# zhanggefan/mmdet3d-gaussian

Measured on AMD Instinct MI355X. Metric: M box-pairs/sec (fwd+bwd) for GWD/KLD/BCD @10M pairs, higher is better.
Workload: dtype f32; 1 GPU; 10000000 synthetic anchor x gt 7-dof box pairs per GPU (BASELINE configs[2]); step = gwd3d + kld3d + bd3d, each GDLoss forward + backward over the whole batch (one plain backward() of the summed losses; fun=log1p, tau=1, reduction=mean, loss_weight=5); pairs_per_gpu=10000000, parallelism=pair-sharded x1, launch=eager, gc_disabled=True, input_allocation=one torch allocation per array, device=MI355X (HIP kernels)

## Files before the change

### include/gd3d.h

```cpp
#ifndef GD3D_H_
#define GD3D_H_

#include <stddef.h>
#include <stdint.h>

#ifdef __cplusplus
extern "C" {
#endif

#define GD3D_ABI_VERSION 6

#define GD3D_E_BADARG 10001
#define GD3D_E_TOOLARGE 10002
#define GD3D_E_HOST 10003

enum {
  GD3D_GWD3D = 0,
  GD3D_KLD3D = 1,
  GD3D_BD3D = 2,
  GD3D_JD3D = 3,
  GD3D_KLD3D_SYMMAX = 4,
  GD3D_KLD3D_SYMMIN = 5,
  GD3D_KFIOU3D = 6,
  GD3D_NUM_LOSS_TYPES = 7
// ... 113 lines not shown
                           int32_t n_l1, float* losses, void* workspace, void* stream);
int gd3d_center_head_keys(int32_t num_tasks, int64_t max_n, int64_t* byte_offset, int64_t* byte_stride);
int gd3d_center_head_finish(const gd3d_params* params, const gd3d_prologue* coder,
                            const gd3d_center_task* tasks, int32_t num_tasks, const float* code_weights,
                            int32_t n_l1, float* losses, void* workspace, const int64_t* order,
                            void* stream);

int gd3d_loss_fused_select(const gd3d_params* params, const gd3d_prologue* prologue, const float* pred,
                           const float* target, const float* weight7, int64_t n, float scale,
                           float* loss_sum, int32_t* any_positive, float* grad_pred, float* grad_target,
                           void* workspace, void* stream, void* start_event, void* stop_event);

int64_t gd3d_one_launch_max_n(void);
int gd3d_loss_fused_one_launch(const gd3d_params* params, const gd3d_prologue* prologue, const float* pred,
                               const float* target, const float* row_weight, const float* weight7, int64_t n,
                               float scale, float* loss_sum, int32_t* any_positive, float* grad_pred,
                               float* grad_target, void* workspace, int32_t* ticket, void* stream);

size_t gd3d_loss_fused_multi_workspace_bytes(int32_t count, int64_t n);
int gd3d_loss_fused_multi_eligible(const gd3d_params* params);
int gd3d_loss_fused_multi(int32_t count, const gd3d_params* params, const float* const* preds, const float* target,
                          int64_t n, const float* scales, float* const* loss_sums, float* const* grad_preds,
                          void* workspace, void* stream);

int gd3d_grad_finish(float* grad_pred, float* grad_target, const float* g, int64_t n,
                     const int32_t* any_positive, const float* weight7, const float* pred,
                     const gd3d_prologue* prologue, void* stream);

int gd3d_probe_stream(const float* x, const float* y, float* z, int64_t n_floats, void* stream,
                      void* start_event, void* stop_event);

int coder_center_decode(const gd3d_prologue* coder, const float* locs, const float* preds, int64_t n,
                        int32_t c, int32_t correct_yaw, float* out, int32_t* num_rot_parity, void* stream);

int coder_center_decode_backward(const gd3d_prologue* coder, const float* grad_out, const float* out,
                                 const int32_t* num_rot_parity, int64_t n, int32_t c,
                                 float* grad_preds, void* stream);

int coder_center_encode(const float* boxes, int64_t n, int32_t c, float* out, void* stream);

int coder_point_decode(const float* priors, const float* preds, int64_t n, int32_t c, int32_t correct_yaw, float* out,
                       int32_t* num_rot_parity, void* stream);
int coder_point_decode_backward(const float* priors, const float* grad_out, const float* out,
                                const int32_t* num_rot_parity, int64_t n, int32_t c, float* grad_preds, void* stream);

int coder_roi_decode(const float* rois, int32_t roi_stride, int32_t first_col, const float* bbox_pred, int64_t n,
// ... 445 lines not shown
```

### mmdet3d-gaussian_amd/_lib.py

```python
import ctypes
import os

from . import build as _build

_lib = None


class Params(ctypes.Structure):
    _fields_ = [('loss_type', ctypes.c_int32), ('fun', ctypes.c_int32),
                ('tau', ctypes.c_float), ('alpha', ctypes.c_float),
                ('center_offset', ctypes.c_float * 3), ('flag', ctypes.c_int32)]


class Prologue(ctypes.Structure):
    _fields_ = [('kind', ctypes.c_int32), ('norm_bbox', ctypes.c_int32), ('aux', ctypes.c_void_p),
                ('out_size_factor', ctypes.c_float), ('voxel_size', ctypes.c_float * 2),
                ('pc_range', ctypes.c_float * 2), ('reserved', ctypes.c_float)]


def fill_geometry(struct, coder):
    struct.norm_bbox = int(bool(coder.norm_bbox))
    struct.out_size_factor = float(coder.out_size_factor)
    struct.voxel_size = (ctypes.c_float * 2)(float(coder.voxel_size[0]), float(coder.voxel_size[1]))
    struct.pc_range = (ctypes.c_float * 2)(float(coder.pc_range[0]), float(coder.pc_range[1]))
# ... 74 lines not shown
                ('gt_start', ctypes.c_int32 * 65), ('pos_iou_thr', ctypes.c_float * 16), ('neg_iou_thr', ctypes.c_float * 16),
                ('min_pos_iou', ctypes.c_float * 16), ('pos_weight', ctypes.c_float), ('dir_offset', ctypes.c_float)]


_vp, _i64, _f32, _int, _sz = ctypes.c_void_p, ctypes.c_int64, ctypes.c_float, ctypes.c_int, ctypes.c_size_t
_i32 = ctypes.c_int32
SYMBOLS = {
    'gd3d_loss_workspace_bytes': (_sz, [_i64]),
    'gd3d_loss_fused': (_int, [ctypes.POINTER(Params), _vp, _vp, _vp, _i64, _f32, _vp, _vp, _vp, _vp, _vp, _vp]),
    'gd3d_loss_fused_w7': (_int, [ctypes.POINTER(Params), _vp, _vp, _vp, _vp, _i64, _f32, _vp, _vp, _vp, _vp, _vp, _vp]),
    'gd3d_loss_fused_decoded': (_int, [ctypes.POINTER(Params), ctypes.POINTER(Prologue), _vp, _vp, _vp, _vp, _i64, _f32,
                                       _vp, _vp, _vp, _vp, _vp, _vp]),
    'gd3d_loss_fused_timed': (_int, [ctypes.POINTER(Params), ctypes.POINTER(Prologue), _vp, _vp, _vp, _vp, _i64, _f32,
                                     _vp, _vp, _vp, _vp, _vp, _vp, _vp, _vp]),
    'gd3d_loss_fused_select': (_int, [ctypes.POINTER(Params), ctypes.POINTER(Prologue), _vp, _vp, _vp, _i64, _f32, _vp, _vp,
                                      _vp, _vp, _vp, _vp, _vp, _vp]),
    'gd3d_one_launch_max_n': (_i64, []),
    'gd3d_loss_fused_one_launch': (_int, [ctypes.POINTER(Params), ctypes.POINTER(Prologue), _vp, _vp, _vp, _vp, _i64, _f32, _vp, _vp,
                                          _vp, _vp, _vp, _vp, _vp]),
    'gd3d_loss_fused_multi_workspace_bytes': (_sz, [_i32, _i64]),
    'gd3d_loss_fused_multi_eligible': (_int, [ctypes.POINTER(Params)]),
    'gd3d_loss_fused_multi': (_int, [_i32, ctypes.POINTER(Params), ctypes.POINTER(_vp), _vp, _i64, ctypes.POINTER(_f32),
                                     ctypes.POINTER(_vp), ctypes.POINTER(_vp), _vp, _vp]),
    'gd3d_loss_fused_cpu': (_int, [ctypes.POINTER(Params), _vp, _vp, _vp, _vp, _i64, _f32, _vp, _vp, _vp, _vp, _vp, ctypes.c_int32]),
    'gd3d_loss_reduce_cpu': (_int, [_vp, _i64, _vp]),
    'gd3d_scale_rows_cpu': (_int, [_vp, _vp, _int, _i64, ctypes.c_int32]),
    'riou_bev_xyxyr_cpu': (_int, [_vp, _i64, _vp, _i64, _vp, ctypes.c_int32]),
    'riou_eval_bev_cpu': (_int, [_vp, _i64, _vp, _i64, _vp, ctypes.c_int32]),
    'riou_eval_3d_cpu': (_int, [_vp, _i64, _vp, _i64, _f32, _vp, ctypes.c_int32]),
    'riou_eval_trans_bev_cpu': (_int, [_vp, _i64, ctypes.c_int32, _vp, _i64, ctypes.c_int32, _vp, ctypes.c_int32]),
    'rnms_bev_cpu': (_int, [_vp, _i64, _f32, _vp, _vp]),
    'rnms_normal_bev_cpu': (_int, [_vp, _i64, _f32, _vp, _vp]),
    'gd3d_grad_finish': (_int, [_vp, _vp, _vp, _i64, _vp, _vp, _vp, ctypes.POINTER(Prologue), _vp]),
    'gd3d_probe_stream': (_int, [_vp, _vp, _vp, _i64, _vp, _vp, _vp]),
    'gd3d_prof_event_create': (_int, [ctypes.POINTER(_vp)]),
    'gd3d_prof_event_destroy': (_int, [_vp]),
    'gd3d_prof_event_elapsed_ms': (_int, [_vp, _vp, ctypes.POINTER(ctypes.c_float)]),
    'gd3d_anchor_head_loss': (_int, [ctypes.POINTER(Params), _vp, ctypes.c_int32, ctypes.c_int32, ctypes.c_int32,
                                     ctypes.c_int32, _vp, _vp, ctypes.POINTER(ctypes.c_float), _vp, _vp, _i64, _f32, _vp,
                                     _vp, _vp, _vp]),
    'gd3d_anchor_head_loss_dense': (_int, [ctypes.POINTER(Params), _vp, ctypes.c_int32, ctypes.c_int32, ctypes.c_int32,
                                           ctypes.c_int32, _vp, _vp, ctypes.POINTER(ctypes.c_float), _vp, _vp,
                                           ctypes.c_int32, _f32, _vp, _vp, _vp, _vp]),
    'gd3d_anchor_head_bbox_loss': (_int, [ctypes.POINTER(Params), ctypes.POINTER(SmoothL1), _vp, ctypes.c_int32,
                                          ctypes.c_int32, ctypes.c_int32, ctypes.c_int32, _vp, _vp,
                                          ctypes.POINTER(ctypes.c_float), _vp, _vp, _i64, _vp, ctypes.c_int32, _f32, _vp,
# ... 421 lines not shown
```

### mmdet3d-gaussian_amd/build.py

```python
import concurrent.futures
import hashlib
import os
import shutil
import subprocess

PKG_DIR = os.path.dirname(os.path.abspath(__file__))
CSRC = os.path.join(PKG_DIR, 'csrc')
LIB_PATH = os.path.join(PKG_DIR, 'libgd3d.so')
ARCH = 'gfx950'

SOURCES = {
    'gd3d_loss.hip': ['-fno-hip-fp32-correctly-rounded-divide-sqrt', '-ffp-contract=fast'],
    'gd3d_anchor_head.hip': ['-fno-hip-fp32-correctly-rounded-divide-sqrt', '-ffp-contract=fast'],
    'gd3d_center_head.hip': ['-fno-hip-fp32-correctly-rounded-divide-sqrt', '-ffp-contract=fast'],
    'rbox.hip': ['-ffp-contract=off'],
    'voxel_scatter.hip': [],
    'device_sort.hip': [],
    'voxel_index.hip': [],
    'eval_match.hip': ['-ffp-contract=off'],
    'coders.hip': ['-ffp-contract=off'],
    'vsa.hip': ['-ffp-contract=off'],
    'pib.hip': ['-ffp-contract=off'],
    'roi_head.hip': ['-ffp-contract=off'],
    'roi_sample.hip': ['-ffp-contract=off'],
# ... 132 lines not shown
          main_objs
    r = subprocess.run(cmd, capture_output=True, text=True)
    if r.returncode != 0:
        raise RuntimeError(f'link failed:\n{r.stderr[-4000:]}')
    os.replace(tmp, LIB_PATH)
    tmp = f'{EXTRAS_PATH}.{os.getpid()}.tmp'
    cmd = [hipcc, '--offload-arch=' + ARCH, '-shared', '-fPIC', '-pthread', '-o', tmp] + extra_objs + \
          ['-L' + PKG_DIR, '-l:libgd3d.so', '-Wl,-rpath,$ORIGIN']
    r = subprocess.run(cmd, capture_output=True, text=True)
    if r.returncode != 0:
        raise RuntimeError(f'link of libgd3d_extras.so failed:\n{r.stderr[-4000:]}')
    os.replace(tmp, EXTRAS_PATH)
    with open(HASH_PATH + f'.{os.getpid()}', 'w') as f:
        f.write(source_hash())
    os.replace(HASH_PATH + f'.{os.getpid()}', HASH_PATH)
    shutil.rmtree(objdir, ignore_errors=True)
    return LIB_PATH


def node_source_hash():
    import torch
    h = hashlib.sha256()
    h.update(torch.__version__.encode())
    for d in (os.path.join(CSRC, NODE_SOURCE), os.path.join(PKG_DIR, '..', 'include', 'gd3d.h')):
        with open(d, 'rb') as f:
            h.update(f.read())
    h.update(repr(node_command('OUT', cxx='CXX')).encode())
    return h.hexdigest()


def node_command(out, cxx=None):
    import sysconfig
    import torch
    tdir = os.path.dirname(os.path.abspath(torch.__file__))
    tlib = os.path.join(tdir, 'lib')
    return [cxx or host_cxx_path(), '-std=c++17', '-O2', '-fPIC', '-shared', '-Wall', '-Wno-unused-function',
            '-D__HIP_PLATFORM_AMD__=1', '-DUSE_ROCM=1', '-DTORCH_EXTENSION_NAME=_gd3d_node',
            f'-D_GLIBCXX_USE_CXX11_ABI={int(torch._C._GLIBCXX_USE_CXX11_ABI)}',
            '-isystem', os.path.join(tdir, 'include'), '-isystem', os.path.join(tdir, 'include', 'torch', 'csrc', 'api', 'include'),
            '-isystem', '/opt/rocm/include', '-isystem', sysconfig.get_paths()['include'],
            os.path.join(CSRC, NODE_SOURCE), '-o', out,
            '-L' + tlib, '-ltorch', '-ltorch_cpu', '-lc10', '-lc10_hip', '-ltorch_hip', '-ltorch_python', '-ldl',
            '-Wl,-rpath,' + tlib]


def node_is_stale():
    if not os.path.isfile(NODE_PATH) or not os.path.isfile(NODE_HASH_PATH):
# ... 28 lines not shown
```

### mmdet3d-gaussian_amd/csrc/gd3d_loss.hip

```cpp
#include <hip/hip_ext.h>

#include <mutex>
#include <unordered_map>

#include "gd3d_loss_common.h"

namespace gd3d {

constexpr int TILE = 256;
constexpr int TILE_F = TILE * 7;
constexpr int TILE_V4 = TILE_F / 4;
constexpr int NPIECE = TILE_F / 256;
constexpr int NWAVE = TILE / 64;

typedef __attribute__((address_space(3))) void lds_ptr_t;
typedef const __attribute__((address_space(1))) void gbl_cptr_t;

constexpr int DMA_AUX = 2;
constexpr int DMA_AUX_TARGET = 0;
constexpr int MIN_LDS = 27300;
constexpr int MIN_LDS_GWD = 32768;
constexpr int MIN_LDS_W7 = 32768;
constexpr int MIN_LDS_KLD = MIN_LDS;
constexpr int MIN_LDS_BD = MIN_LDS;
// ... 440 lines not shown
    double s2 = 0.0;
#pragma unroll
    for (int k = 0; k < 16; ++k) s2 += sd[tid * 16 + k];
#pragma unroll
    for (int off = 32; off >= 1; off >>= 1) s2 += __shfl_down(s2, off, 64);
    if (tid == 0) *out = (float)s2;
  }
}
__global__ __launch_bounds__(1024) void reduce_partials_kernel(const float* __restrict__ partials, long long nb,
                                                               float* __restrict__ out) {
  __shared__ double sd[1024];
  reduce_partials_body(partials, nb, out, sd);
}
struct ReduceMultiArgs {
  float* out[MULTI_MAX];
};
__global__ __launch_bounds__(1024) void reduce_partials_multi_kernel(const float* __restrict__ partials, long long nb,
                                                                     long long nbp, const ReduceMultiArgs o) {
  __shared__ double sd[1024];
  float* out = o.out[0];
  if (blockIdx.x == 1) out = o.out[1];
  if (blockIdx.x == 2) out = o.out[2];
  reduce_partials_body(partials + (long long)blockIdx.x * nbp, nb, out, sd);
}
int reduce_partials(const float* partials, long long nb, float* out, hipStream_t s) {
  hipLaunchKernelGGL(reduce_partials_kernel, dim3(1), dim3(1024), 0, s, partials, nb, out);
  return (int)hipGetLastError();
}

__global__ __launch_bounds__(1024) void scale_rows_kernel(float* __restrict__ grad, const float* __restrict__ g,
                                                         int per_row, long long nflt) {
  float gs = 1.0f;
  if (!per_row) {
    gs = g[0];
    if (gs == 1.0f) return;
  }
  const long long stride = (long long)gridDim.x * blockDim.x;
  const long long i0 = (long long)blockIdx.x * blockDim.x + threadIdx.x;
  if (!per_row && (((uintptr_t)grad & 15) == 0)) {
    v4f* g4 = reinterpret_cast<v4f*>(grad);
    const long long nv = nflt >> 2;
    for (long long i = i0; i < nv; i += stride) g4[i] = g4[i] * gs;
    for (long long i = (nv << 2) + i0; i < nflt; i += stride) grad[i] *= gs;
    return;
  }
  for (long long i = i0; i < nflt; i += stride) grad[i] *= per_row ? g[i / 7] : gs;
// ... 359 lines not shown
  hipExtLaunchKernelGGL(probe_add_kernel, dim3((unsigned)nb), dim3(PROBE_T), 0u, (hipStream_t)stream, (hipEvent_t)start_event,
                        (hipEvent_t)stop_event, 0u, (const v4f*)x, (const v4f*)y, (v4f*)z, nv);
  return (int)hipGetLastError();
}

int gd3d_loss_reduce(const void* workspace, int64_t n, float* loss_sum, void* stream) {
  if (n < 0 || loss_sum == nullptr) return GD3D_E_BADARG;
  hipStream_t s = (hipStream_t)stream;
  if (n == 0) return fill_words(loss_sum, sizeof(float), 0u, s);
  if (workspace == nullptr) return GD3D_E_BADARG;
  const long long nparts = (n + TILE - 1) / TILE;
  return reduce_partials((const float*)workspace, nparts, loss_sum, s);
}

size_t gd3d_loss_fused_multi_workspace_bytes(int32_t count, int64_t n) {
  if (n <= 0 || count <= 0) return 64;
  return (size_t)(4 * (int64_t)count * ws_nbp(n) + 16);
}

int gd3d_loss_fused_multi_eligible(const gd3d_params* p) {
  return p != nullptr && multi_marked(p->loss_type, p->fun, p->flag != 0) ? 1 : 0;
}

int gd3d_loss_fused_multi(int32_t count, const gd3d_params* params, const float* const* preds, const float* target,
                          int64_t n, const float* scales, float* const* loss_sums, float* const* grad_preds,
                          void* workspace, void* stream) {
  if (count < 2 || count > MULTI_MAX || params == nullptr || preds == nullptr || scales == nullptr || loss_sums == nullptr ||
      n < 0)
    return GD3D_E_BADARG;
  for (int k = 0; k < count; ++k) {
    if (!gd3d_loss_fused_multi_eligible(&params[k]) || loss_sums[k] == nullptr) return GD3D_E_BADARG;
    if (n > 0 && preds[k] == nullptr) return GD3D_E_BADARG;
  }
  hipStream_t s = (hipStream_t)stream;
  if (n == 0) {
    for (int k = 0; k < count; ++k) {
      const int e0 = fill_words(loss_sums[k], sizeof(float), 0u, s);
      if (e0 != 0) return e0;
    }
    return 0;
  }
  if (target == nullptr || workspace == nullptr || ((uintptr_t)workspace & 15) != 0) return GD3D_E_BADARG;
  const int64_t nb = (n + TILE - 1) / TILE;
  if (nb > 0x7fffffffLL) return GD3D_E_TOOLARGE;
  int order[MULTI_MAX] = {0, 1, 2};
  for (int i = 1; i < count; ++i)
    for (int j = i; j > 0 && params[order[j]].loss_type < params[order[j - 1]].loss_type; --j) {
      const int t = order[j];
      order[j] = order[j - 1];
      order[j - 1] = t;
    }
  const long long nbp = ws_nbp(n);
  MultiArgs a = {};
  ReduceMultiArgs r = {};
  uintptr_t bits = (uintptr_t)target;
  int lt[MULTI_MAX] = {-1, -1, -1};
  for (int j = 0; j < count; ++j) {
    const int k = order[j];
    const gd3d_params& p = params[k];
    lt[j] = p.loss_type;
// ... 3 lines not shown
    a.scale[j] = scales[k];
    a.alpha[j] = p.alpha;
    a.ia2[j] = gd3d_inv_alpha2(p.alpha);
    a.tau[j] = p.tau;
    for (int q = 0; q < 3; ++q) a.c[j][q] = p.center_offset[q];
    r.out[j] = loss_sums[k];
    bits |= (uintptr_t)a.pred[j] | (uintptr_t)a.gp[j];
  }
  a.target = target;
  a.n = n;
  a.vec_ok = (bits & 15) == 0;
  bool reuse = false;
  next_tile_order_reversed(s, nullptr, -1, &reuse);
  const hipError_t e = with_multi_tuple(lt[0], lt[1], lt[2], [&](auto tup) {
    using T = decltype(tup);
    constexpr int K = T::count;
    size_t lds = (size_t)((K + 1) * TILE_F + 32) * sizeof(float);
    constexpr size_t min_lds = K == 3 ? MULTI_LDS_K3 : MULTI_LDS_K2;
    if (lds < min_lds) lds = min_lds;
    hipLaunchKernelGGL((fused_multi_kernel<T::l0, T::l1, T::l2>), dim3((unsigned)nb), dim3(TILE), lds, s, a);
    return hipGetLastError();
  });
  if (e != hipSuccess) return (int)e;
  hipLaunchKernelGGL(reduce_partials_multi_kernel, dim3((unsigned)count), dim3(1024), 0, s, (const float*)workspace,
                     (long long)nb, nbp, r);
  return (int)hipGetLastError();
}

int gd3d_prof_event_create(void** event) {
  if (event == nullptr) return GD3D_E_BADARG;
  hipEvent_t e = nullptr;
  const hipError_t rc = hipEventCreate(&e);
  *event = (void*)e;
  return (int)rc;
}

int gd3d_prof_event_destroy(void* event) {
  if (event == nullptr) return 0;
  return (int)hipEventDestroy((hipEvent_t)event);
}

int gd3d_prof_event_elapsed_ms(void* start_event, void* stop_event, float* ms) {
  if (start_event == nullptr || stop_event == nullptr || ms == nullptr) return GD3D_E_BADARG;
  return (int)hipEventElapsedTime(ms, (hipEvent_t)start_event, (hipEvent_t)stop_event);
}

int gd3d_scale_rows(float* grad, const float* g, int per_row, int64_t n, void* stream) {
  if (n < 0 || (n > 0 && (grad == nullptr || g == nullptr))) return GD3D_E_BADARG;
  if (n == 0) return 0;
// ... 15 lines not shown
```

### mmdet3d-gaussian_amd/csrc/torch_node.cpp

```cpp
#include <torch/extension.h>
#include <torch/csrc/autograd/functions/basic_ops.h>
#include <torch/csrc/autograd/functions/utils.h>
#include <torch/csrc/autograd/saved_variable.h>
#include <c10/hip/HIPStream.h>
#include <ATen/Parallel.h>

#include <dlfcn.h>

#include <atomic>
#include <chrono>
#include <cstring>
#include <exception>
#include <limits>
#include <mutex>
#include <sstream>
#include <vector>

#include "../../include/gd3d.h"

namespace {

using at::Tensor;
using torch::autograd::variable_list;

struct Abi {
  decltype(&::gd3d_loss_fused_decoded) loss_fused_decoded = nullptr;
  decltype(&::gd3d_loss_fused_timed) loss_fused_timed = nullptr;
  decltype(&::gd3d_loss_fused_select) loss_fused_select = nullptr;
  decltype(&::gd3d_loss_fused_one_launch) loss_fused_one_launch = nullptr;
  decltype(&::gd3d_loss_fused_multi) loss_fused_multi = nullptr;
  decltype(&::gd3d_loss_fused_multi_eligible) loss_fused_multi_eligible = nullptr;
  decltype(&::gd3d_loss_fused_multi_workspace_bytes) loss_fused_multi_workspace_bytes = nullptr;
  decltype(&::gd3d_grad_finish) grad_finish = nullptr;
  decltype(&::gd3d_loss_fused_cpu) loss_fused_cpu = nullptr;
  decltype(&::gd3d_scale_rows_cpu) scale_rows_cpu = nullptr;
  decltype(&::gd3d_abi_version) abi_version = nullptr;
  decltype(&::rnms_scored) nms_scored = nullptr;
  decltype(&::gd3d_anchor_head_bbox_loss) anchor_head = nullptr;
  decltype(&::gd3d_anchor_head_bbox_loss_dyn) anchor_head_dyn = nullptr;
  decltype(&::gd3d_scale_rows) scale_rows = nullptr;
  decltype(&::gd3d_loss_workspace_bytes) loss_workspace_bytes = nullptr;
  decltype(&::vox_scatter_reduce) scatter_reduce = nullptr;
  decltype(&::vox_scatter_backward) scatter_backward = nullptr;
  decltype(&::vox_scatter_backward_grouped) scatter_backward_grouped = nullptr;
  decltype(&::rnms_scored_workspace_bytes) nms_scored_workspace_bytes = nullptr;
  bool bound = false;
} abi;

template <typename F>
void resolve(void* image, const char* name, F& slot) {
  slot = reinterpret_cast<F>(dlsym(image, name));
  TORCH_CHECK(slot != nullptr, "gd3d node: libgd3d.so does not export ", name);
}

int bind(const std::string& path) {
  void* image = dlopen(path.c_str(), RTLD_NOW | RTLD_LOCAL);
  TORCH_CHECK(image != nullptr, "gd3d node: cannot open ", path, ": ", dlerror());
  resolve(image, "gd3d_loss_fused_decoded", abi.loss_fused_decoded);
  resolve(image, "gd3d_loss_fused_timed", abi.loss_fused_timed);
  resolve(image, "gd3d_loss_fused_select", abi.loss_fused_select);
  resolve(image, "gd3d_loss_fused_one_launch", abi.loss_fused_one_launch);
  resolve(image, "gd3d_loss_fused_multi", abi.loss_fused_multi);
  resolve(image, "gd3d_loss_fused_multi_eligible", abi.loss_fused_multi_eligible);
  resolve(image, "gd3d_loss_fused_multi_workspace_bytes", abi.loss_fused_multi_workspace_bytes);
  resolve(image, "gd3d_grad_finish", abi.grad_finish);
  resolve(image, "gd3d_loss_fused_cpu", abi.loss_fused_cpu);
  resolve(image, "gd3d_scale_rows_cpu", abi.scale_rows_cpu);
  resolve(image, "gd3d_abi_version", abi.abi_version);
  resolve(image, "rnms_scored", abi.nms_scored);
  resolve(image, "gd3d_anchor_head_bbox_loss", abi.anchor_head);
  resolve(image, "gd3d_anchor_head_bbox_loss_dyn", abi.anchor_head_dyn);
  resolve(image, "gd3d_scale_rows", abi.scale_rows);
  resolve(image, "gd3d_loss_workspace_bytes", abi.loss_workspace_bytes);
  resolve(image, "vox_scatter_reduce", abi.scatter_reduce);
  resolve(image, "vox_scatter_backward", abi.scatter_backward);
  resolve(image, "vox_scatter_backward_grouped", abi.scatter_backward_grouped);
  resolve(image, "rnms_scored_workspace_bytes", abi.nms_scored_workspace_bytes);
  const int version = abi.abi_version(nullptr);
  TORCH_CHECK(version == GD3D_ABI_VERSION, "gd3d node: built against ABI ", GD3D_ABI_VERSION, ", the library reports ", version);
  abi.bound = true;
  return version;
}

std::atomic<int64_t> g_finish_calls{0};

// ... 116 lines not shown
      auto err = std::make_shared<torch::autograd::DelayedError>(
          "trying to differentiate twice a function that was marked with @once_differentiable", (int64_t)alias.size());
      at::AutoGradMode grad_on(true);
      return (*err)(std::move(alias));
    }
    return out;
  }
};

using ImplPtr = c10::intrusive_ptr<c10::TensorImpl, c10::UndefinedTensorImpl>;
using WeakImpl = c10::weak_intrusive_ptr<c10::TensorImpl, c10::UndefinedTensorImpl>;
struct PendingEntry {
  explicit PendingEntry(const Tensor& loss) : total(loss.getIntrusivePtr()) {}
  WeakImpl total;
  std::weak_ptr<ReducedBackward> node;
  bool has_node = false;
  Tensor pred, target;
  uint32_t pred_version = 0, target_version = 0;
  float* gp = nullptr;
  float* base = nullptr;
  gd3d_params params;
  float scale = 1.0f;
};
struct PendingList {
  c10::Device device{c10::kCPU};
  void* stream = nullptr;
  const float* target = nullptr;
  int64_t n = 0;
  std::vector<PendingEntry> entries;
};
std::mutex g_pending_mu;
std::vector<PendingList> g_pending;
std::atomic<int64_t> g_multi_launches{0}, g_single_launches{0}, g_dropped{0};

void flush_list(PendingList& pl) {
  std::vector<PendingEntry> entries = std::move(pl.entries);
  pl.entries.clear();
  struct Live {
    PendingEntry* e;
    ImplPtr total;
    std::shared_ptr<ReducedBackward> node;
  };
  std::vector<Live> good, bad;
  std::string why;
  for (PendingEntry& e : entries) {
    Live l{&e, e.total.lock(), e.node.lock()};
    if (l.node) l.node->pending_.store(false, std::memory_order_release);
    if (!l.total.defined() || (e.has_node && !l.node)) {
      g_dropped.fetch_add(1, std::memory_order_relaxed);
      continue;
    }
    const bool pred_ok = e.pred._version() == e.pred_version, target_ok = e.target._version() == e.target_version;
    if (pred_ok && target_ok) {
      good.push_back(std::move(l));
      continue;
    }
    if (why.empty()) {
      const Tensor& t = pred_ok ? e.target : e.pred;
      std::ostringstream os;
      os << "GDLoss: one of the variables needed by a deferred loss evaluation has been modified by an inplace operation: ["
         << t.toString() << " " << t.sizes() << "] (" << (pred_ok ? "target" : "pred") << ") is at version " << t._version()
         << "; expected version " << (pred_ok ? e.target_version : e.pred_version)
         << " instead. Hint: call gd_loss.flush() before editing an input in place, or set GD3D_DEFER=0.";
      why = os.str();
    }
    bad.push_back(std::move(l));
  }
  c10::OptionalDeviceGuard device_guard;
  if (!good.empty() || !bad.empty()) device_guard.reset_device(pl.device);
  if (good.size() == 1) {
    PendingEntry& e = *good[0].e;
    g_single_launches.fetch_add(1, std::memory_order_relaxed);
    fail(abi.loss_fused_timed(&e.params, nullptr, fp(e.pred), fp(e.target), nullptr, nullptr, pl.n, e.scale, nullptr, e.base, e.gp,
                               nullptr, e.base + 4, pl.stream, nullptr, nullptr), "gd3d_loss_fused_timed");
  } else if (good.size() >= 2) {
    const int32_t k = (int32_t)good.size();
    gd3d_params params[3];
    const float* preds[3];
    float scales[3];
    float* sums[3];
    float* gps[3];
    for (int32_t i = 0; i < k; ++i) {
      const PendingEntry& e = *good[i].e;
      params[i] = e.params;
      preds[i] = fp(e.pred);
      scales[i] = e.scale;
      sums[i] = e.base;
      gps[i] = e.gp;
    }
    g_multi_launches.fetch_add(1, std::memory_order_relaxed);
    fail(abi.loss_fused_multi(k, params, preds, pl.target, pl.n, scales, sums, gps, good[0].e->base + 4, pl.stream),
         "gd3d_loss_fused_multi");
  }
  if (!bad.empty()) {
    at::AutoDispatchBelowADInplaceOrView below_autograd;
    for (Live& l : bad) {
      if (l.node) l.node->poisoned_ = true;
      Tensor(l.total).fill_(std::numeric_limits<float>::quiet_NaN());
    }
    TORCH_CHECK(false, why);
  }
}

void flush_pending() {
  std::lock_guard<std::mutex> lock(g_pending_mu);
  std::vector<PendingList> lists = std::move(g_pending);
  g_pending.clear();
  std::exception_ptr first;
  for (PendingList& pl : lists) {
    try {
      if (!pl.entries.empty()) flush_list(pl);
    } catch (...) {
      if (!first) first = std::current_exception();
    }
  }
  if (first) std::rethrow_exception(first);
}

void enqueue_pending(PendingEntry&& e, const c10::Device& device, void* stream, int64_t n) {
  std::lock_guard<std::mutex> lock(g_pending_mu);
  PendingList* pl = nullptr;
  for (PendingList& l : g_pending)
    if (l.device == device && l.stream == stream) pl = &l;
  if (pl == nullptr) {
    if (g_pending.size() >= 64) {
      std::vector<PendingList> lists = std::move(g_pending);
      g_pending.clear();
      for (PendingList& l : lists)
        if (!l.entries.empty()) flush_list(l);
    }
    g_pending.emplace_back();
    pl = &g_pending.back();
    pl->device = device;
    pl->stream = stream;
  }
  if (!pl->entries.empty()) {
    bool fits = pl->target == fp(e.target) && pl->n == n && pl->entries.size() < 3;
    for (const PendingEntry& q : pl->entries) fits = fits && fp(q.pred) != fp(e.pred);
    if (!fits) flush_list(*pl);
  }
  pl->target = fp(e.target);
  pl->n = n;
  pl->entries.push_back(std::move(e));
  if (pl->entries.size() == 3) flush_list(*pl);
}

std::tuple<Tensor, c10::optional<Tensor>> reduced(const Tensor& pred, const Tensor& target, const c10::optional<Tensor>& weight,
                                                  int64_t params_addr, int64_t prologue_addr, const c10::optional<Tensor>& aux,
                                                  double scale, bool select, int64_t ticket, int64_t ev_start, int64_t ev_stop,
                                                  int64_t ws_floats, bool want_flag, bool defer) {
  TORCH_CHECK(pred.dim() == 2 && pred.size(1) == 7 && pred.scalar_type() == at::kFloat && pred.is_contiguous() &&
                  target.sizes() == pred.sizes() && target.scalar_type() == at::kFloat && target.is_contiguous() &&
                  target.device() == pred.device(),
              "gd3d node: pred / target must be contiguous fp32 (N, 7) tensors on one device");
  TORCH_CHECK(pred.is_cuda() || pred.is_cpu(), "gd3d node: no implementation for device ", pred.device());
  if (pred.is_cpu()) require_cpu_twins();
  TORCH_CHECK(abi.bound, "gd3d node: bind(path of libgd3d.so) has not been called");
  const int64_t n = pred.size(0);
  Tensor w;
  if (weight.has_value() && weight->defined()) {
    w = *weight;
    TORCH_CHECK(w.scalar_type() == at::kFloat && w.is_contiguous() && w.device() == pred.device() && w.size(0) == n &&
                    (w.dim() == 1 || (w.dim() == 2 && w.size(1) == 7)),
                "gd3d node: weight must be a contiguous fp32 (N,) or (N, 7) tensor on pred's device");
  }
  TORCH_CHECK(!select || (w.defined() && w.dim() == 2 && pred.is_cuda()), "gd3d node: select needs an (N, 7) weight on the GPU");
  TORCH_CHECK(prologue_addr == 0 || pred.is_cuda(), "GDLoss: the head-level fusions (bbox-coder prologue) are GPU-only");
// ... 367 lines not shown
  TORCH_CHECK(k != PENDING, "nms_gpu: the NMS kernels finished without reporting a count");
  TORCH_CHECK(k >= 0, "nms_gpu: the device-side NMS scan gave up (num_keep = ", k, "); the result is void");
  if (post_max >= 0 && k > post_max) k = post_max;
  return {keep.narrow(0, 0, k), Tensor()};
}

void set_unit_grad(int64_t device_index, int64_t address) {
  TORCH_CHECK(device_index < MAX_DEVICES, "gd3d node: device index ", device_index);
  const int slot = device_index < 0 ? MAX_DEVICES : (int)device_index;
  g_unit_grad[slot] = (const void*)address;
}

}

PYBIND11_MODULE(_gd3d_node, m) {
  m.doc() = "C++ autograd node of GDLoss's reduced forms above the C ABI of libgd3d.so";
  m.def("reduced", &reduced, py::arg("pred"), py::arg("target"), py::arg("weight"), py::arg("params"), py::arg("prologue"),
        py::arg("aux"), py::arg("scale"), py::arg("select"), py::arg("ticket"), py::arg("ev_start"), py::arg("ev_stop"),
        py::arg("ws_floats"), py::arg("want_flag"), py::arg("defer") = false);
  m.def("flush_pending", &flush_pending, py::call_guard<py::gil_scoped_release>(),
        "launch every deferred GDLoss forward (one fused launch per list of two or three losses on one target)");
  m.def("pending_stats", []() { return std::make_tuple(g_multi_launches.load(), g_single_launches.load(), g_dropped.load()); },
        "(multi-loss launches, single launches, dropped entries) made by flushes so far");
  m.def("nms_scored", &nms_scored, py::arg("boxes"), py::arg("scores"), py::arg("thresh"), py::arg("n_keep"), py::arg("normal"),
        py::arg("padded"), py::arg("post_max"));
  m.def("anchor_head", &anchor_head, py::arg("bbox_pred"), py::arg("bbox_targets"), py::arg("bbox_weights"), py::arg("anchors"),
        py::arg("sel"), py::arg("params"), py::arg("sl1"), py::arg("decode_weight"), py::arg("dense"), py::arg("num_classes"),
        py::arg("scale"), py::arg("avg_dev"), py::arg("w_gd"), py::arg("w_sl1"));
  m.def("scatter_reduce", &scatter_reduce, py::arg("feats"), py::arg("point2voxel_map"), py::arg("voxel_points_count"), py::arg("reduce"),
        py::arg("order"), py::arg("seg"));
  m.def("set_unit_grad", &set_unit_grad);
  m.def("finish_calls", []() { return g_finish_calls.load(); }, "gd3d_grad_finish launches made by backward so far");
  m.def("bind", &bind, "resolve the C ABI from the loaded libgd3d.so; returns its ABI version");
}
```

### mmdet3d-gaussian_amd/gd_loss.py

```python
import ctypes
import os
from copy import deepcopy

import torch
from torch import nn
from . import _host, _lib
from ._host import guard_double_backward, unit_grad
from .registry import LOSSES, register_with_mmdet

LOSS_TYPES = {'gwd3d': 0, 'kld3d': 1, 'bd3d': 2, 'jd3d': 3, 'kld3d_symmax': 4, 'kld3d_symmin': 5, 'kfiou3d': 6}
FUNS = {'none': 0, 'log1p': 1, 'expm1': 2, 'nlog': 3}

PROFILE_EVENTS = None


class DispatchTimer:
    __slots__ = ('start', 'stop', '_abi')

    def __init__(self):
        self.start = self.stop = None
        self._abi = _library()
        for slot in ('start', 'stop'):
            h = ctypes.c_void_p()
            _lib.check(self._abi.gd3d_prof_event_create(ctypes.byref(h)), 'gd3d_prof_event_create')
# ... 79 lines not shown
        pool[1] += 1
        return pool[0].data_ptr() + 16 * (pool[1] - 1)
    t = _TICKETS.get((dev_index, stream))
    if t is None:
        if len(_TICKETS) > 256:
            _TICKETS.clear()
        dev = torch.device('cuda', dev_index)
        t = _TICKETS[(dev_index, stream)] = torch.zeros(4, dtype=torch.int32, device=dev)
        if dev_index not in _GRAPH_TICKETS:
            _GRAPH_TICKETS[dev_index] = [torch.zeros(4 * _GRAPH_SLOTS, dtype=torch.int32, device=dev), 0]
    return t.data_ptr()


_ws_floats = _host.memo(lambda n: _library().gd3d_loss_workspace_bytes(n) // 4)


_UNIT_ROOT = os.environ.get('GD3D_UNIT_ROOT', '1') != '0'
_TENSOR_BACKWARD = torch.Tensor.backward


_DEFER = os.environ.get('GD3D_DEFER', '1') != '0'
DEFER_MIN_N = 32768
_deferred = False


def flush():
    global _deferred
    _deferred = False
    fn = getattr(_lib._node, 'flush_pending', None)
    if fn is not None:
        fn()


class LossValue(torch.Tensor):

    @classmethod
    def __torch_function__(cls, func, types, args=(), kwargs=None):
        if _deferred:
            flush()
        if func is _TENSOR_BACKWARD and _UNIT_ROOT:
            kw = dict(kwargs) if kwargs else {}
            self = args[0]
            gradient = kw.pop('gradient', args[1] if len(args) > 1 else None)
            if (gradient is None and self.dim() == 0 and self.dtype == torch.float32 and self.requires_grad and
                    (self.is_cuda or self.device.type == 'cpu')):
                names = ('retain_graph', 'create_graph', 'inputs')
                for k, v in zip(names, args[2:]):
                    kw.setdefault(k, v)
                with torch._C.DisableTorchFunctionSubclass():
                    return torch.autograd.backward(self, unit_grad(self.device), kw.get('retain_graph'),
                                                   kw.get('create_graph', False), inputs=kw.get('inputs'))
        return super().__torch_function__(func, types, args, kwargs)


    def __deepcopy__(self, memo):
        return self.as_subclass(torch.Tensor).__deepcopy__(memo).as_subclass(LossValue)


def _as_loss_value(t):
    if _UNIT_ROOT and type(t) is torch.Tensor:
        if not _host.has_unit_grad(t):
# ... 196 lines not shown
```

Baseline: 99360 M box-pairs/s.

## Fold deferred loss additions into the multi-loss reduction kernel

Additions between deferred GDLoss values (the summed gwd+kld+bd losses) are captured as pending sums instead of forcing a flush. Their results are computed in a new single-block reduction kernel that also reduces the per-loss partials with double-buffered float4 loads. This removes the separate elementwise add launches and the Python-side flush on the first add. The auto-flush at three entries is removed, so lists flush only on demand. This adds a custom autograd node and weak-reference bookkeeping, with some risk if callers relied on the eager flush.

```diff
diff --git a/include/gd3d.h b/include/gd3d.h
--- a/include/gd3d.h
+++ b/include/gd3d.h
@@ -159,6 +159,12 @@
 int gd3d_loss_fused_multi(int32_t count, const gd3d_params* params, const float* const* preds, const float* target,
                           int64_t n, const float* scales, float* const* loss_sums, float* const* grad_preds,
                           void* workspace, void* stream);
+
+#define GD3D_MULTI_MAX_SUMS 4
+int gd3d_loss_fused_multi_sums(int32_t count, const gd3d_params* params, const float* const* preds, const float* target,
+                               int64_t n, const float* scales, float* const* loss_sums, float* const* grad_preds,
+                               int32_t nsum, const int32_t* lhs, const int32_t* rhs, float* const* sum_out,
+                               void* workspace, void* stream);
 
 int gd3d_grad_finish(float* grad_pred, float* grad_target, const float* g, int64_t n,
                      const int32_t* any_positive, const float* weight7, const float* pred,
diff --git a/mmdet3d-gaussian_amd/_lib.py b/mmdet3d-gaussian_amd/_lib.py
--- a/mmdet3d-gaussian_amd/_lib.py
+++ b/mmdet3d-gaussian_amd/_lib.py
@@ -120,6 +120,9 @@
     'gd3d_loss_fused_multi_eligible': (_int, [ctypes.POINTER(Params)]),
     'gd3d_loss_fused_multi': (_int, [_i32, ctypes.POINTER(Params), ctypes.POINTER(_vp), _vp, _i64, ctypes.POINTER(_f32),
                                      ctypes.POINTER(_vp), ctypes.POINTER(_vp), _vp, _vp]),
+    'gd3d_loss_fused_multi_sums': (_int, [_i32, ctypes.POINTER(Params), ctypes.POINTER(_vp), _vp, _i64, ctypes.POINTER(_f32),
+                                          ctypes.POINTER(_vp), ctypes.POINTER(_vp), _i32, ctypes.POINTER(_i32), ctypes.POINTER(_i32),
+                                          ctypes.POINTER(_vp), _vp, _vp]),
     'gd3d_loss_fused_cpu': (_int, [ctypes.POINTER(Params), _vp, _vp, _vp, _vp, _i64, _f32, _vp, _vp, _vp, _vp, _vp, ctypes.c_int32]),
     'gd3d_loss_reduce_cpu': (_int, [_vp, _i64, _vp]),
     'gd3d_scale_rows_cpu': (_int, [_vp, _vp, _int, _i64, ctypes.c_int32]),
diff --git a/mmdet3d-gaussian_amd/build.py b/mmdet3d-gaussian_amd/build.py
--- a/mmdet3d-gaussian_amd/build.py
+++ b/mmdet3d-gaussian_amd/build.py
@@ -178,7 +178,7 @@
     import torch
     h = hashlib.sha256()
     h.update(torch.__version__.encode())
-    for d in (os.path.join(CSRC, NODE_SOURCE), os.path.join(PKG_DIR, '..', 'include', 'gd3d.h')):
+    for d in (os.path.join(CSRC, NODE_SOURCE), os.path.join(CSRC, 'sum_fold.h'), os.path.join(PKG_DIR, '..', 'include', 'gd3d.h')):
         with open(d, 'rb') as f:
             h.update(f.read())
     h.update(repr(node_command('OUT', cxx='CXX')).encode())
diff --git a/mmdet3d-gaussian_amd/csrc/gd3d_loss.hip b/mmdet3d-gaussian_amd/csrc/gd3d_loss.hip
--- a/mmdet3d-gaussian_amd/csrc/gd3d_loss.hip
+++ b/mmdet3d-gaussian_amd/csrc/gd3d_loss.hip
@@ -486,6 +486,94 @@
   if (blockIdx.x == 1) out = o.out[1];
   if (blockIdx.x == 2) out = o.out[2];
   reduce_partials_body(partials + (long long)blockIdx.x * nbp, nb, out, sd);
+}
+constexpr int MULTI_MAX_SUMS = GD3D_MULTI_MAX_SUMS;
+struct ReduceSumsArgs {
+  float* out[MULTI_MAX];
+  float* sum_out[MULTI_MAX_SUMS];
+  int lhs[MULTI_MAX_SUMS], rhs[MULTI_MAX_SUMS];
+  int nsum;
+};
+constexpr int SUMS_RU = 12;
+GD_DEV void sums_load_chunk(float4 (&v)[SUMS_RU], const float* __restrict__ partials, long long nbp, long long nv, long long rounds,
+                            long long c, int tid) {
+  const long long k = c / rounds, i0 = (c - k * rounds) * (1024 * SUMS_RU);
+  const float4* p4 = reinterpret_cast<const float4*>(partials + k * nbp);
+#pragma unroll
+  for (int u = 0; u < SUMS_RU; ++u) {
+    const long long i = i0 + (long long)u * 1024 + tid;
+    v[u] = i < nv ? p4[i] : make_float4(0.f, 0.f, 0.f, 0.f);
+  }
+}
+template <int K>
+GD_DEV void sums_add_chunk(const float4 (&v)[SUMS_RU], double (&acc)[K], long long rounds, long long c) {
+  const int k = (int)(c / rounds);
+  double a = k == 0 ? acc[0] : (k == 1 ? acc[1] : acc[K - 1]);
+#pragma unroll
+  for (int u = 0; u < SUMS_RU; ++u) a += ((double)v[u].x + (double)v[u].y) + ((double)v[u].z + (double)v[u].w);
+  if (k == 0) acc[0] = a;
+  else if (k == 1) acc[1] = a;
+  else acc[K - 1] = a;
+}
+template <int K>
+__global__ __launch_bounds__(1024) void reduce_partials_sums_kernel(const float* __restrict__ partials, long long nb,
+                                                                    long long nbp, const ReduceSumsArgs o) {
+  __shared__ double sd[K][1024];
+  __shared__ float sval[MULTI_MAX + MULTI_MAX_SUMS];
+  const int tid = threadIdx.x;
+  const long long nv = nb >> 2;
+  const long long rounds = (nv + 1024 * SUMS_RU - 1) / (1024 * SUMS_RU);
+  const long long total = K * rounds;
+  const long long tail = (nv << 2) + tid;
+  float tv[K];
+#pragma unroll
+  for (int k = 0; k < K; ++k) tv[k] = tail < nb ? partials[k * nbp + tail] : 0.0f;
+  double acc[K];
+#pragma unroll
+  for (int k = 0; k < K; ++k) acc[k] = 0.0;
+  float4 va[SUMS_RU], vb[SUMS_RU];
+  long long c = 0;
+  if (total > 0) sums_load_chunk(va, partials, nbp, nv, rounds, 0, tid);
+  while (c < total) {
+    if (c + 1 < total) sums_load_chunk(vb, partials, nbp, nv, rounds, c + 1, tid);
+    sums_add_chunk<K>(va, acc, rounds, c);
+    if (++c >= total) break;
+    if (c + 1 < total) sums_load_chunk(va, partials, nbp, nv, rounds, c + 1, tid);
+    sums_add_chunk<K>(vb, acc, rounds, c);
+    ++c;
+  }
+#pragma unroll
+  for (int k = 0; k < K; ++k) {
+    if (tail < nb) acc[k] += (double)tv[k];
+    sd[k][tid] = acc[k];
+  }
+  __syncthreads();
+  const int wave = tid >> 6, lane = tid & 63;
+  if (wave < K) {
+    double s2 = 0.0;
+#pragma unroll
+    for (int k = 0; k < 16; ++k) s2 += sd[wave][lane * 16 + k];
+#pragma unroll
+    for (int off = 32; off >= 1; off >>= 1) s2 += __shfl_down(s2, off, 64);
+    if (lane == 0) {
+      const float r = (float)s2;
+      float* out = o.out[0];
+      if (wave == 1) out = o.out[1];
+      if (wave == 2) out = o.out[K - 1];
+      *out = r;
+      sval[wave] = r;
+    }
+  }
+  __syncthreads();
+  if (tid == 0) {
+#pragma unroll
+    for (int i = 0; i < MULTI_MAX_SUMS; ++i) {
+      if (i >= o.nsum) break;
+      const float r = sval[o.lhs[i]] + sval[o.rhs[i]];
+      sval[K + i] = r;
+      *o.sum_out[i] = r;
+    }
+  }
 }
 int reduce_partials(const float* partials, long long nb, float* out, hipStream_t s) {
   hipLaunchKernelGGL(reduce_partials_kernel, dim3(1), dim3(1024), 0, s, partials, nb, out);
@@ -891,9 +979,9 @@
   return p != nullptr && multi_marked(p->loss_type, p->fun, p->flag != 0) ? 1 : 0;
 }
 
-int gd3d_loss_fused_multi(int32_t count, const gd3d_params* params, const float* const* preds, const float* target,
-                          int64_t n, const float* scales, float* const* loss_sums, float* const* grad_preds,
-                          void* workspace, void* stream) {
+static int multi_launch(int32_t count, const gd3d_params* params, const float* const* preds, const float* target, int64_t n,
+                        const float* scales, float* const* loss_sums, float* const* grad_preds, int32_t nsum, const int32_t* lhs,
+                        const int32_t* rhs, float* const* sum_out, void* workspace, void* stream) {
   if (count < 2 || count > MULTI_MAX || params == nullptr || preds == nullptr || scales == nullptr || loss_sums == nullptr ||
       n < 0)
     return GD3D_E_BADARG;
@@ -901,10 +989,14 @@
     if (!gd3d_loss_fused_multi_eligible(&params[k]) || loss_sums[k] == nullptr) return GD3D_E_BADARG;
     if (n > 0 && preds[k] == nullptr) return GD3D_E_BADARG;
   }
+  if (nsum < 0 || nsum > MULTI_MAX_SUMS || (nsum > 0 && (lhs == nullptr || rhs == nullptr || sum_out == nullptr)))
+    return GD3D_E_BADARG;
+  for (int i = 0; i < nsum; ++i)
+    if (lhs[i] < 0 || lhs[i] >= count + i || rhs[i] < 0 || rhs[i] >= count + i || sum_out[i] == nullptr) return GD3D_E_BADARG;
   hipStream_t s = (hipStream_t)stream;
   if (n == 0) {
-    for (int k = 0; k < count; ++k) {
-      const int e0 = fill_words(loss_sums[k], sizeof(float), 0u, s);
+    for (int k = 0; k < count + nsum; ++k) {
+      const int e0 = fill_words(k < count ? loss_sums[k] : sum_out[k - count], sizeof(float), 0u, s);
       if (e0 != 0) return e0;
     }
     return 0;
@@ -954,9 +1046,40 @@
     return hipGetLastError();
   });
   if (e != hipSuccess) return (int)e;
-  hipLaunchKernelGGL(reduce_partials_multi_kernel, dim3((unsigned)count), dim3(1024), 0, s, (const float*)workspace,
-                     (long long)nb, nbp, r);
+  if (nsum == 0) {
+    hipLaunchKernelGGL(reduce_partials_multi_kernel, dim3((unsigned)count), dim3(1024), 0, s, (const float*)workspace,
+                       (long long)nb, nbp, r);
+    return (int)hipGetLastError();
+  }
+  int inv[MULTI_MAX] = {0, 1, 2};
+  for (int j = 0; j < count; ++j) inv[order[j]] = j;
+  ReduceSumsArgs q = {};
+  for (int j = 0; j < count; ++j) q.out[j] = r.out[j];
+  for (int i = 0; i < nsum; ++i) {
+    q.lhs[i] = lhs[i] < count ? inv[lhs[i]] : lhs[i];
+    q.rhs[i] = rhs[i] < count ? inv[rhs[i]] : rhs[i];
+    q.sum_out[i] = sum_out[i];
+  }
+  q.nsum = nsum;
+  if (count == 2)
+    hipLaunchKernelGGL(reduce_partials_sums_kernel<2>, dim3(1), dim3(1024), 0, s, (const float*)workspace, (long long)nb, nbp, q);
+  else
+    hipLaunchKernelGGL(reduce_partials_sums_kernel<3>, dim3(1), dim3(1024), 0, s, (const float*)workspace, (long long)nb, nbp, q);
   return (int)hipGetLastError();
+}
+
+int gd3d_loss_fused_multi(int32_t count, const gd3d_params* params, const float* const* preds, const float* target,
+                          int64_t n, const float* scales, float* const* loss_sums, float* const* grad_preds,
+                          void* workspace, void* stream) {
+  return multi_launch(count, params, preds, target, n, scales, loss_sums, grad_preds, 0, nullptr, nullptr, nullptr, workspace,
+                      stream);
+}
+
+int gd3d_loss_fused_multi_sums(int32_t count, const gd3d_params* params, const float* const* preds, const float* target,
+                               int64_t n, const float* scales, float* const* loss_sums, float* const* grad_preds,
+                               int32_t nsum, const int32_t* lhs, const int32_t* rhs, float* const* sum_out, void* workspace,
+                               void* stream) {
+  return multi_launch(count, params, preds, target, n, scales, loss_sums, grad_preds, nsum, lhs, rhs, sum_out, workspace, stream);
 }
 
 int gd3d_prof_event_create(void** event) {
diff --git a/mmdet3d-gaussian_amd/csrc/sum_fold.h b/mmdet3d-gaussian_amd/csrc/sum_fold.h
--- /dev/null
+++ b/mmdet3d-gaussian_amd/csrc/sum_fold.h
@@ -0,0 +1,43 @@
+#pragma once
+#include <cstddef>
+#include <cstdint>
+#include <vector>
+
+namespace sum_fold {
+
+template <class Alive, class Release>
+std::vector<size_t> prune_dead_sums(size_t nsum, Alive&& alive, Release&& release) {
+  std::vector<size_t> live;
+  for (size_t i = nsum; i-- > 0;) {
+    if (alive(i)) live.push_back(i);
+    else release(i);
+  }
+  return std::vector<size_t>(live.rbegin(), live.rend());
+}
+
+struct SumKeys {
+  const void* out;
+  const void* lhs;
+  const void* rhs;
+};
+
+inline bool remap_sums(const std::vector<const void*>& losses, const std::vector<SumKeys>& sums, std::vector<int32_t>& lhs,
+                       std::vector<int32_t>& rhs) {
+  auto index_of = [&](const void* key, size_t before) -> int32_t {
+    for (size_t k = 0; k < losses.size(); ++k)
+      if (losses[k] == key) return (int32_t)k;
+    for (size_t j = 0; j < before; ++j)
+      if (sums[j].out == key) return (int32_t)(losses.size() + j);
+    return -1;
+  };
+  lhs.assign(sums.size(), -1);
+  rhs.assign(sums.size(), -1);
+  for (size_t i = 0; i < sums.size(); ++i) {
+    lhs[i] = index_of(sums[i].lhs, i);
+    rhs[i] = index_of(sums[i].rhs, i);
+    if (lhs[i] < 0 || rhs[i] < 0) return false;
+  }
+  return true;
+}
+
+}
diff --git a/mmdet3d-gaussian_amd/csrc/torch_node.cpp b/mmdet3d-gaussian_amd/csrc/torch_node.cpp
--- a/mmdet3d-gaussian_amd/csrc/torch_node.cpp
+++ b/mmdet3d-gaussian_amd/csrc/torch_node.cpp
@@ -17,6 +17,7 @@
 #include <vector>
 
 #include "../../include/gd3d.h"
+#include "sum_fold.h"
 
 namespace {
 
@@ -29,6 +30,7 @@
   decltype(&::gd3d_loss_fused_select) loss_fused_select = nullptr;
   decltype(&::gd3d_loss_fused_one_launch) loss_fused_one_launch = nullptr;
   decltype(&::gd3d_loss_fused_multi) loss_fused_multi = nullptr;
+  decltype(&::gd3d_loss_fused_multi_sums) loss_fused_multi_sums = nullptr;
   decltype(&::gd3d_loss_fused_multi_eligible) loss_fused_multi_eligible = nullptr;
   decltype(&::gd3d_loss_fused_multi_workspace_bytes) loss_fused_multi_workspace_bytes = nullptr;
   decltype(&::gd3d_grad_finish) grad_finish = nullptr;
@@ -61,6 +63,7 @@
   resolve(image, "gd3d_loss_fused_select", abi.loss_fused_select);
   resolve(image, "gd3d_loss_fused_one_launch", abi.loss_fused_one_launch);
   resolve(image, "gd3d_loss_fused_multi", abi.loss_fused_multi);
+  resolve(image, "gd3d_loss_fused_multi_sums", abi.loss_fused_multi_sums);
   resolve(image, "gd3d_loss_fused_multi_eligible", abi.loss_fused_multi_eligible);
   resolve(image, "gd3d_loss_fused_multi_workspace_bytes", abi.loss_fused_multi_workspace_bytes);
   resolve(image, "gd3d_grad_finish", abi.grad_finish);
@@ -223,20 +226,40 @@
   gd3d_params params;
   float scale = 1.0f;
 };
+struct PendingSum {
+  PendingSum(const Tensor& result, const Tensor& a, const Tensor& b) : out(result.getIntrusivePtr()), lhs(a), rhs(b) {}
+  WeakImpl out;
+  Tensor lhs, rhs;
+};
+constexpr size_t MAX_PENDING_SUMS = GD3D_MULTI_MAX_SUMS;
 struct PendingList {
   c10::Device device{c10::kCPU};
   void* stream = nullptr;
   const float* target = nullptr;
   int64_t n = 0;
   std::vector<PendingEntry> entries;
+  std::vector<PendingSum> sums;
 };
 std::mutex g_pending_mu;
 std::vector<PendingList> g_pending;
-std::atomic<int64_t> g_multi_launches{0}, g_single_launches{0}, g_dropped{0};
+std::atomic<int64_t> g_multi_launches{0}, g_single_launches{0}, g_dropped{0}, g_folded_sums{0};
 
 void flush_list(PendingList& pl) {
   std::vector<PendingEntry> entries = std::move(pl.entries);
   pl.entries.clear();
+  std::vector<PendingSum> sums = std::move(pl.sums);
+  pl.sums.clear();
+  std::vector<ImplPtr> sum_out(sums.size());
+  const std::vector<size_t> live_sums = sum_fold::prune_dead_sums(
+      sums.size(),
+      [&](size_t i) {
+        sum_out[i] = sums[i].out.lock();
+        return sum_out[i].defined();
+      },
+      [&](size_t i) {
+        sums[i].lhs = Tensor();
+        sums[i].rhs = Tensor();
+      });
   struct Live {
     PendingEntry* e;
     ImplPtr total;
@@ -267,8 +290,18 @@
     }
     bad.push_back(std::move(l));
   }
+  std::vector<int32_t> lhs, rhs;
+  bool fold = !live_sums.empty() && good.size() >= 2 && bad.empty();
+  if (fold) {
+    std::vector<const void*> losses;
+    for (const Live& l : good) losses.push_back(l.total.get());
+    std::vector<sum_fold::SumKeys> keys;
+    for (size_t i : live_sums)
+      keys.push_back({sum_out[i].get(), sums[i].lhs.unsafeGetTensorImpl(), sums[i].rhs.unsafeGetTensorImpl()});
+    fold = sum_fold::remap_sums(losses, keys, lhs, rhs);
+  }
   c10::OptionalDeviceGuard device_guard;
-  if (!good.empty() || !bad.empty()) device_guard.reset_device(pl.device);
+  if (!good.empty() || !bad.empty() || !live_sums.empty()) device_guard.reset_device(pl.device);
   if (good.size() == 1) {
     PendingEntry& e = *good[0].e;
     g_single_launches.fetch_add(1, std::memory_order_relaxed);
@@ -279,19 +312,27 @@
     gd3d_params params[3];
     const float* preds[3];
     float scales[3];
-    float* sums[3];
+    float* totals[3];
     float* gps[3];
     for (int32_t i = 0; i < k; ++i) {
       const PendingEntry& e = *good[i].e;
       params[i] = e.params;
       preds[i] = fp(e.pred);
       scales[i] = e.scale;
-      sums[i] = e.base;
+      totals[i] = e.base;
       gps[i] = e.gp;
     }
     g_multi_launches.fetch_add(1, std::memory_order_relaxed);
-    fail(abi.loss_fused_multi(k, params, preds, pl.target, pl.n, scales, sums, gps, good[0].e->base + 4, pl.stream),
-         "gd3d_loss_fused_multi");
+    if (fold) {
+      float* outs[MAX_PENDING_SUMS];
+      for (size_t j = 0; j < live_sums.size(); ++j) outs[j] = Tensor(sum_out[live_sums[j]]).data_ptr<float>();
+      fail(abi.loss_fused_multi_sums(k, params, preds, pl.target, pl.n, scales, totals, gps, (int32_t)live_sums.size(), lhs.data(),
+                                      rhs.data(), outs, good[0].e->base + 4, pl.stream), "gd3d_loss_fused_multi_sums");
+      g_folded_sums.fetch_add((int64_t)live_sums.size(), std::memory_order_relaxed);
+    } else {
+      fail(abi.loss_fused_multi(k, params, preds, pl.target, pl.n, scales, totals, gps, good[0].e->base + 4, pl.stream),
+           "gd3d_loss_fused_multi");
+    }
   }
   if (!bad.empty()) {
     at::AutoDispatchBelowADInplaceOrView below_autograd;
@@ -299,8 +340,23 @@
       if (l.node) l.node->poisoned_ = true;
       Tensor(l.total).fill_(std::numeric_limits<float>::quiet_NaN());
     }
-    TORCH_CHECK(false, why);
-  }
+  }
+  if (!fold && !live_sums.empty()) {
+    at::AutoDispatchBelowADInplaceOrView below_autograd;
+    const c10::hip::HIPStream mine = c10::hip::getCurrentHIPStream(pl.device.index());
+    c10::hip::setCurrentHIPStream(c10::hip::getStreamFromExternal((hipStream_t)pl.stream, pl.device.index()));
+    try {
+      for (size_t i : live_sums) {
+        Tensor out(sum_out[i]);
+        at::add_out(out, sums[i].lhs, sums[i].rhs);
+      }
+    } catch (...) {
+      c10::hip::setCurrentHIPStream(mine);
+      throw;
+    }
+    c10::hip::setCurrentHIPStream(mine);
+  }
+  TORCH_CHECK(bad.empty(), why);
 }
 
 void flush_pending() {
@@ -316,6 +372,46 @@
     }
   }
   if (first) std::rethrow_exception(first);
+}
+
+struct PendingSumBackward : public torch::autograd::Node {
+  std::string name() const override { return "GDLossSumBackward"; }
+  variable_list apply(variable_list&& grads) override { return {grads[0], grads[0]}; }
+};
+
+c10::optional<Tensor> add_pending(const Tensor& a, const Tensor& b) {
+  if (!a.defined() || !b.defined() || !a.is_cuda() || !b.is_cuda()) return c10::nullopt;
+  std::lock_guard<std::mutex> lock(g_pending_mu);
+  const c10::TensorImpl* const ia = a.unsafeGetTensorImpl();
+  const c10::TensorImpl* const ib = b.unsafeGetTensorImpl();
+  for (PendingList& pl : g_pending) {
+    if (pl.entries.empty()) continue;
+    auto member = [&](const c10::TensorImpl* t) {
+      for (const PendingEntry& e : pl.entries)
+        if (e.total._unsafe_get_target() == t) return true;
+      for (const PendingSum& s : pl.sums)
+        if (s.out._unsafe_get_target() == t) return true;
+      return false;
+    };
+    const bool has_a = member(ia), has_b = member(ib);
+    if (!has_a && !has_b) continue;
+    if (!has_a || !has_b || pl.sums.size() >= MAX_PENDING_SUMS) return c10::nullopt;
+    if ((void*)c10::hip::getCurrentHIPStream(pl.device.index()).stream() != pl.stream) return c10::nullopt;
+    Tensor out;
+    {
+      at::AutoDispatchBelowADInplaceOrView below_autograd;
+      c10::DeviceGuard device_guard(pl.device);
+      out = at::empty({}, a.options());
+    }
+    if (at::GradMode::is_enabled() && (a.requires_grad() || b.requires_grad())) {
+      auto node = std::shared_ptr<PendingSumBackward>(new PendingSumBackward(), torch::autograd::deleteNode);
+      node->set_next_edges(torch::autograd::collect_next_edges(a, b));
+      torch::autograd::set_history(out, node);
+    }
+    pl.sums.emplace_back(out, a, b);
+    return out;
+  }
+  return c10::nullopt;
 }
 
 void enqueue_pending(PendingEntry&& e, const c10::Device& device, void* stream, int64_t n) {
@@ -343,7 +439,6 @@
   pl->target = fp(e.target);
   pl->n = n;
   pl->entries.push_back(std::move(e));
-  if (pl->entries.size() == 3) flush_list(*pl);
 }
 
 std::tuple<Tensor, c10::optional<Tensor>> reduced(const Tensor& pred, const Tensor& target, const c10::optional<Tensor>& weight,
@@ -757,6 +852,9 @@
         "launch every deferred GDLoss forward (one fused launch per list of two or three losses on one target)");
   m.def("pending_stats", []() { return std::make_tuple(g_multi_launches.load(), g_single_launches.load(), g_dropped.load()); },
         "(multi-loss launches, single launches, dropped entries) made by flushes so far");
+  m.def("add_pending", &add_pending, py::arg("a"), py::arg("b"), py::call_guard<py::gil_scoped_release>(),
+        "a + b of two values queued on one list, written by that list's flush (None: not both pending, or no room: flush and add)");
+  m.def("folded_sums", []() { return g_folded_sums.load(); }, "queued sums written by a multi-loss second-stage launch so far");
   m.def("nms_scored", &nms_scored, py::arg("boxes"), py::arg("scores"), py::arg("thresh"), py::arg("n_keep"), py::arg("normal"),
         py::arg("padded"), py::arg("post_max"));
   m.def("anchor_head", &anchor_head, py::arg("bbox_pred"), py::arg("bbox_targets"), py::arg("bbox_weights"), py::arg("anchors"),
diff --git a/mmdet3d-gaussian_amd/gd_loss.py b/mmdet3d-gaussian_amd/gd_loss.py
--- a/mmdet3d-gaussian_amd/gd_loss.py
+++ b/mmdet3d-gaussian_amd/gd_loss.py
@@ -125,6 +125,8 @@
 _DEFER = os.environ.get('GD3D_DEFER', '1') != '0'
 DEFER_MIN_N = 32768
 _deferred = False
+_TENSOR_RADD = torch.Tensor.__radd__
+_FOLDED_ADDS = frozenset((torch.add, torch.Tensor.add, torch.Tensor.__add__, _TENSOR_RADD))
 
 
 def flush():
@@ -140,6 +142,12 @@
     @classmethod
     def __torch_function__(cls, func, types, args=(), kwargs=None):
         if _deferred:
+            if func in _FOLDED_ADDS and not kwargs and len(args) == 2 and type(args[0]) is LossValue and type(args[1]) is LossValue:
+                add = getattr(_lib._node, 'add_pending', None)
+                if add is not None:
+                    out = add(args[1], args[0]) if func is _TENSOR_RADD else add(args[0], args[1])
+                    if out is not None:
+                        return _as_loss_value(out)
             flush()
         if func is _TENSOR_BACKWARD and _UNIT_ROOT:
             kw = dict(kwargs) if kwargs else {}
```

Measured after the change: 98050 M box-pairs/s. 0.987x the previous value.
